# rokulkarni15/distributed-llm-training-inference

Measured on AMD Instinct MI355X. Metric: train tok/s Llama-2-7B ZeRO-3+LoRA at 1/2/4/8 GPUs; serve tok/s + p50 TTFT, higher is better.
Workload: dtype bf16

## Files before the change

### lumen/csrc/binding.cpp

```cpp
#include <torch/extension.h>
#include <c10/hip/HIPStream.h>
#include <hip/hip_runtime.h>

#include <algorithm>
#include <optional>
#include <stdexcept>
#include <string>
#include <vector>

extern "C" {
hipError_t lumen_rmsnorm_fwd(int, const void*, const void*, const void*, void*, void*, float*, int,
                             int, float, hipStream_t);
hipError_t lumen_rmsnorm_bwd(int, const void*, const void*, const void*, const float*, const void*,
                             void*, float*, int, int, hipStream_t);
hipError_t lumen_qkv_rope(int, int, void*, void*, void*, void*, const int*, const float*,
                          const float*, int, int, int, int, int, hipStream_t);
hipError_t lumen_rope_inplace(int, void*, const int*, const float*, const float*, int, int, int,
                              int, hipStream_t);
hipError_t lumen_swiglu(int, int, const void*, const void*, void*, int, int, int, int, hipStream_t);
hipError_t lumen_scale_dev(int, void*, long long, const float*, const float*, hipStream_t);
hipError_t lumen_cross_entropy(int, void*, const int64_t*, float*, float*, int, int, int, float,
                               int, const float*, hipStream_t);
hipError_t lumen_grad_norm_sq(int, const void*, long long, float*, hipStream_t);
hipError_t lumen_adamw(float*, int, const void*, float*, float*, int, void*, long long, float, float,
// ... 606 lines not shown
                    big.data_ptr(), ldb, small.data_ptr<float>(), lds, out.data_ptr(), cs0,
                    cs1, static_cast<float>(alpha), static_cast<int>(T), static_cast<int>(J),
                    static_cast<int>(split), static_cast<unsigned long long>(seed),
                    static_cast<unsigned int>(drop_thresh), static_cast<float>(drop_scale),
                    drop_ld, drop_col0, nseg, bo, so, oo, nc,
                    rope_cos ? rope_cos->data_ptr<float>() : nullptr,
                    rope_sin ? rope_sin->data_ptr<float>() : nullptr,
                    rope_pos ? rope_pos->data_ptr<int>() : nullptr, static_cast<int>(rope_mask),
                    cur_stream()),
        "lora2");
}

bool is_fp8(const at::Tensor& t) { return t.scalar_type() == at::kFloat8_e4m3fn; }

void need_cuda_f32(const at::Tensor& t, const char* what) {
  if (!t.is_cuda() || t.scalar_type() != at::kFloat)
    throw std::invalid_argument(std::string("lumen: ") + what + " must be an f32 GPU tensor");
}

void lora3_down(const at::Tensor& x, int64_t ldx, const at::Tensor& A, at::Tensor& Z, int64_t ldz,
                int64_t T, int64_t K, int64_t R, double alpha, int64_t seed, int64_t thresh,
                double drop_scale, int64_t drop_ld, int64_t drop_col0,
                const c10::optional<at::Tensor>& xe, int64_t xk, int64_t KP,
                const c10::optional<at::Tensor>& cnt, const c10::optional<at::Tensor>& slab) {
  if (!x.is_cuda()) throw std::invalid_argument("lumen: lora3_down needs GPU tensors");
  need_cuda_f32(A, "lora3_down A");
  need_cuda_f32(Z, "lora3_down Z");
  if (A.stride(1) != 1 || A.size(0) < R || A.size(1) < K || x.size(0) < T || Z.size(0) < T)
    throw std::invalid_argument("lumen: lora3_down shape mismatch");
  void* xp = nullptr;
  long long ldxe = 0;
  unsigned* cp = nullptr;
  if (xe && xe->defined()) {
    if (!cnt || !cnt->defined() || cnt->scalar_type() != at::kInt || !cnt->is_cuda() ||
        cnt->numel() < (T + 63) / 64 || xe->scalar_type() != x.scalar_type() || xe->dim() != 2 ||
        xe->stride(1) != 1 || xe->size(0) < T || xe->size(1) < xk + KP || Z.size(1) < R)
      throw std::invalid_argument("lumen: lora3_down fold tail: xe [T, >= xk + KP], cnt int32 [T / 64]");
    xp = xe->data_ptr();
    ldxe = xe->stride(0);
    cp = reinterpret_cast<unsigned*>(cnt->data_ptr<int>());
  }
  float* sp = nullptr;
  if (slab && slab->defined()) {
    const bool with_cnt = cnt && cnt->defined();
    if ((with_cnt && (cnt->scalar_type() != at::kInt || !cnt->is_cuda() ||
                      cnt->numel() < (T + 63) / 64)) ||
        slab->scalar_type() != at::kFloat || !slab->is_cuda() ||
        slab->numel() < ((T + 63) / 64) * ((K + 1023) / 1024) * 64 * R)
      throw std::invalid_argument("lumen: lora3_down slab / cnt too small");
    sp = slab->data_ptr<float>();
    cp = with_cnt ? reinterpret_cast<unsigned*>(cnt->data_ptr<int>()) : nullptr;
  }
  check(lumen_lora3_down(dcode(x), x.data_ptr(), ldx, A.data_ptr<float>(), A.stride(0),
                         Z.data_ptr<float>(), ldz, static_cast<int>(T), static_cast<int>(K),
                         static_cast<int>(R), static_cast<float>(alpha),
                         static_cast<unsigned long long>(seed), static_cast<unsigned int>(thresh),
                         static_cast<float>(drop_scale), drop_ld, drop_col0, xp, ldxe,
                         static_cast<int>(xk), static_cast<int>(KP), cp, sp, cur_stream()),
        "lora3_down");
}

void lora3_up(int64_t fwd, at::Tensor& out, int64_t ldo, const at::Tensor& s1, int64_t ld1,
              const at::Tensor& s2, int64_t ld2, int64_t T, int64_t J, double alpha, int64_t seed,
              int64_t thresh, double drop_scale, int64_t drop_ld, int64_t drop_col0,
              const std::vector<std::vector<int64_t>>& segs, const c10::optional<at::Tensor>& rope_cos,
              const c10::optional<at::Tensor>& rope_sin, const c10::optional<at::Tensor>& rope_pos,
              int64_t rope_mask) {
  if (!out.is_cuda()) throw std::invalid_argument("lumen: lora3_up needs GPU tensors");
  need_cuda_f32(s1, "lora3_up s1");
  need_cuda_f32(s2, "lora3_up s2");
  const int nseg = static_cast<int>(segs.size());
  if (nseg < 1 || nseg > 4) throw std::invalid_argument("lumen: lora3_up needs 1..4 segments");
  long long oo[4] = {0}, so1[4] = {0}, so2[4] = {0};
// ... 555 lines not shown
```

### lumen/csrc/kernels/lora_v3.hip

```cpp
#include "tile128.h"
#include "det.h"

namespace lumen {
namespace lv3 {

using namespace tile;

struct Drop {
  unsigned int seed, thresh;
  float scale;
  long long ld;
  long long col0;
};

__device__ __forceinline__ uint4 mask8(uint4 u, uint32_t keep) {
  const auto wm = [keep](int w) {
    return ((keep >> (2 * w)) & 1u ? 0x0000FFFFu : 0u) | ((keep >> (2 * w + 1)) & 1u ? 0xFFFF0000u : 0u);
  };
  return make_uint4(u.x & wm(0), u.y & wm(1), u.z & wm(2), u.w & wm(3));
}

template <typename T>
__device__ __forceinline__ uint4 ld_f32x8(const float* p, bool ok) {
  if (!ok) return make_uint4(0, 0, 0, 0);
  const float4 u = *reinterpret_cast<const float4*>(p);
  const float4 v = *reinterpret_cast<const float4*>(p + 4);
  return make_uint4(pk2<T>(u.x, u.y), pk2<T>(u.z, u.w), pk2<T>(v.x, v.y), pk2<T>(v.z, v.w));
}

struct DownArgs {
  const void* x; long long ldx;
  const float* A; long long lda;
// ... 325 lines not shown
    for (int i = 0; i < 4; ++i) ycur[i] = ynxt[i];
  }
}

struct DySeg {
  long long n_off[4], r_off[4], b_off[4];
  int n_len[4];
  int nseg;
};

struct DyArgs {
  const void* dy; long long ldy;
  const float* B; int r;
  const float* Z; long long ldz;
  float* dZ; long long lddz;
  float* dB;
  int T, TW;
  float alpha;
  DySeg seg;
  int probe;
  float* slab_z; float* slab_b;
  unsigned* cnt_z; unsigned* cnt_b;
};

constexpr int kDyCC = 2;

template <typename T>
__device__ __forceinline__ void dy_load(uint4 (&v)[4], const T* base, long long ld, int r0, int rmax,
                                        int c0, int cmax) {
#pragma unroll
  for (int i = 0; i < 4; ++i) {
    const int idx = threadIdx.x + i * 256;
    const int r = r0 + (idx >> 4), c = c0 + (idx & 15) * 8;
    const uint4 u = *reinterpret_cast<const uint4*>(base + (long long)min(r, rmax - 1) * ld +
                                                     min(c, cmax - 8));
    v[i] = (r < rmax && c < cmax) ? u : make_uint4(0, 0, 0, 0);
  }
}

__device__ __forceinline__ void dy_store(char* img, const uint4 (&v)[4]) {
#pragma unroll
  for (int i = 0; i < 4; ++i) {
    const int idx = threadIdx.x + i * 256;
    *reinterpret_cast<uint4*>(img + img_off_b(idx >> 4, idx & 15)) = v[i];
  }
}

template <typename T, int NJ>
__global__ void __launch_bounds__(256) dy3_kernel(DyArgs a) {
  __shared__ __attribute__((aligned(16))) char img[2][64 * 256];
  const int seg = blockIdx.z;
  const int NL = a.seg.n_len[seg];
  const int cb = blockIdx.x * 128 * kDyCC;
  const int tb = blockIdx.y * a.TW, te = min(a.T, tb + a.TW);
  if (cb >= NL || tb >= a.T) return;
  const int lane = threadIdx.x & 63, wid = threadIdx.x >> 6, L = lane & 15, g = lane >> 4;
  const T* dy = reinterpret_cast<const T*>(a.dy) + a.seg.n_off[seg];
  const float* B = a.B + a.seg.b_off[seg] * a.r;
  const float* Z = a.Z + a.seg.r_off[seg];
  float* dZ = a.dZ + a.seg.r_off[seg];
  float* dB = a.dB + a.seg.b_off[seg] * a.r;
  const int nch = min(kDyCC, (NL - cb + 127) / 128);

  uint4 bop[kDyCC][4][NJ];
#pragma unroll
  for (int cc = 0; cc < kDyCC; ++cc)
#pragma unroll
    for (int i = 0; i < 4; ++i)
#pragma unroll
      for (int jt = 0; jt < NJ; ++jt) {
        float f[8];
#pragma unroll
        for (int e = 0; e < 8; ++e) {
          const int c = cb + cc * 128 + 32 * i + 8 * g + e;
          const float u = B[(long long)min(c, NL - 1) * a.r + jt * 16 + L];
          f[e] = c < NL ? u : 0.f;
        }
        bop[cc][i][jt] = pack8<T>(f);
      }
  f32x4 dbacc[kDyCC][2][NJ];
#pragma unroll
  for (int cc = 0; cc < kDyCC; ++cc)
#pragma unroll
    for (int m = 0; m < 2; ++m)
#pragma unroll
      for (int jt = 0; jt < NJ; ++jt) dbacc[cc][m][jt] = f32x4{0.f, 0.f, 0.f, 0.f};

  const int nsub = (te - tb + 63) / 64;
  const int nstage = nsub * nch;
  uint4 v[4];
  dy_load<T>(v, dy, a.ldy, tb, te, cb, NL);
  int buf = 0;
  f32x4 dzacc[NJ];
  uint4 zop[2][NJ];
  for (int s = 0; s < nstage; ++s, buf ^= 1) {
    const int ts = s / nch, cc = s % nch;
    const int t0 = tb + ts * 64, cbase = cb + cc * 128;
    dy_store(img[buf], v);
    __syncthreads();
    float zf[2][NJ][8];
#pragma unroll
    for (int ks = 0; ks < 2; ++ks)
#pragma unroll
      for (int jt = 0; jt < NJ; ++jt)
#pragma unroll
        for (int e = 0; e < 8; ++e) {
          const int t = t0 + 32 * ks + 8 * g + e;
          zf[ks][jt][e] = Z[(long long)min(t, te - 1) * a.ldz + jt * 16 + L];
        }
    {
      const int s1 = min(s + 1, nstage - 1);
      const int ts1 = s1 / nch, cc1 = s1 % nch;
      dy_load<T>(v, dy, a.ldy, tb + ts1 * 64, te, cb + cc1 * 128, NL);
    }
    if (cc == 0) {
#pragma unroll
      for (int jt = 0; jt < NJ; ++jt) dzacc[jt] = f32x4{0.f, 0.f, 0.f, 0.f};
    }
    const char* im = img[buf];
#pragma unroll
    for (int i = 0; i < 4; ++i) {
      const uint4 av = row_read_b(im, wid * 16 + L, i * 4 + g);
#pragma unroll
      for (int c2 = 0; c2 < kDyCC; ++c2)
        if (c2 == cc) {
#pragma unroll
          for (int jt = 0; jt < NJ; ++jt) dzacc[jt] = Mfma<T>::run(av, bop[c2][i][jt], dzacc[jt]);
        }
    }
#pragma unroll
    for (int ks = 0; ks < 2; ++ks)
#pragma unroll
      for (int jt = 0; jt < NJ; ++jt) {
        float f[8];
#pragma unroll
        for (int e = 0; e < 8; ++e) f[e] = t0 + 32 * ks + 8 * g + e < te ? zf[ks][jt][e] : 0.f;
        zop[ks][jt] = pack8<T>(f);
      }
#pragma unroll
    for (int ks = 0; ks < 2; ++ks)
#pragma unroll
      for (int m = 0; m < 2; ++m) {
        const uint4 tv = tr_read_img_b(im, ks * 32, wid * 32 + m * 16, lane);
#pragma unroll
        for (int c2 = 0; c2 < kDyCC; ++c2)
          if (c2 == cc) {
#pragma unroll
            for (int jt = 0; jt < NJ; ++jt) dbacc[c2][m][jt] = Mfma<T>::run(tv, zop[ks][jt], dbacc[c2][m][jt]);
          }
      }
    if (cc == nch - 1) {
      if (a.slab_z != nullptr) {
        float* sz = a.slab_z + (((long long)seg * gridDim.y + blockIdx.y) * gridDim.x + blockIdx.x) *
                                   ((long long)a.TW * a.r);
#pragma unroll
        for (int jt = 0; jt < NJ; ++jt)
#pragma unroll
          for (int r = 0; r < 4; ++r) {
            const int t = t0 + wid * 16 + g * 4 + r;
            if (t < te) det::st_wt(sz + (long long)(t - tb) * a.r + jt * 16 + L, dzacc[jt][r]);
          }
      } else {
#pragma unroll
        for (int jt = 0; jt < NJ; ++jt)
#pragma unroll
          for (int r = 0; r < 4; ++r) {
            const int t = t0 + wid * 16 + g * 4 + r;
            if (t < te && (!(a.probe & 16) || dzacc[jt][r] == 1234.5f))
              atomicAdd(dZ + (long long)t * a.lddz + jt * 16 + L, a.alpha * dzacc[jt][r]);
          }
      }
    }
  }
  if (a.slab_z != nullptr) {
    float* sb = a.slab_b + (((long long)seg * gridDim.x + blockIdx.x) * gridDim.y + blockIdx.y) *
                               (256LL * a.r);
#pragma unroll
    for (int cc = 0; cc < kDyCC; ++cc) {
      if (cc >= nch) break;
#pragma unroll
      for (int m = 0; m < 2; ++m)
#pragma unroll
        for (int jt = 0; jt < NJ; ++jt)
#pragma unroll
          for (int r = 0; r < 4; ++r) {
            const int cl = cc * 128 + wid * 32 + m * 16 + g * 4 + r;
            if (cb + cl < NL) det::st_wt(sb + (long long)cl * a.r + jt * 16 + L, dbacc[cc][m][jt][r]);
          }
    }
    if (a.cnt_z == nullptr) return;
    __shared__ int lastf;
    const int ncb = (NL + 128 * kDyCC - 1) / (128 * kDyCC);
    const int J = NJ * 16;
    if (det::last_arriver(a.cnt_z + (long long)seg * gridDim.y + blockIdx.y, ncb, &lastf)) {
      const float* base = a.slab_z + ((long long)seg * gridDim.y + blockIdx.y) * gridDim.x *
                                         ((long long)a.TW * a.r);
      for (int i = threadIdx.x; i < (te - tb) * (J / 2); i += 256) {
        const int tl = i / (J / 2), j = (i % (J / 2)) * 2;
        const float2 v = det::sum_pairs(base + (long long)tl * a.r + j, (long long)a.TW * a.r, ncb);
        float* o = dZ + (long long)(tb + tl) * a.lddz + j;
        o[0] = a.alpha * v.x;
        o[1] = a.alpha * v.y;
      }
    }
    if (det::last_arriver(a.cnt_b + (long long)seg * gridDim.x + blockIdx.x, gridDim.y, &lastf)) {
      const float* base = a.slab_b + ((long long)seg * gridDim.x + blockIdx.x) * gridDim.y *
// ... 61 lines not shown
    const float2 v = sum_pairs_plain(base, (long long)a.TW * a.r, ncb);
    float* o = a.dZ + a.seg.r_off[seg] + t * a.lddz + j;
    o[0] = a.alpha * v.x;
    o[1] = a.alpha * v.y;
  } else {
    const long long c = i / hr;
    if (c >= NL) return;
    const int gx = (int)(c / (128 * kDyCC)), cl = (int)(c % (128 * kDyCC));
    const float* base = a.slab_b + (((long long)seg * gx_n + gx) * gy_n) * (256LL * a.r) +
                        (long long)cl * a.r + j;
    const float2 v = sum_pairs_plain(base, 256LL * a.r, gy_n);
    float* o = a.dB + (a.seg.b_off[seg] + c) * a.r + j;
    o[0] += a.alpha * v.x;
    o[1] += a.alpha * v.y;
  }
}

__global__ void __launch_bounds__(256) dxa3_reduce_kernel(const float* __restrict__ slab,
                                                          float* __restrict__ dA, long long ldda,
                                                          int R, int K, int gy_n, float scale) {
  const long long i = (long long)blockIdx.x * 256 + threadIdx.x;
  const int hk = K / 2;
  if (i >= (long long)R * hk) return;
  const int j = (int)(i / hk), k = (int)(i % hk) * 2;
  const int gx = k / 128, kl = k % 128;
  const float2 v = sum_pairs_plain(slab + ((long long)gx * gy_n) * (128LL * R) +
                                       (long long)j * 128 + kl,
                                   128LL * R, gy_n);
  float* o = dA + (long long)j * ldda + k;
  o[0] += scale * v.x;
  o[1] += scale * v.y;
}

__global__ void __launch_bounds__(256) down3_reduce_kernel(const float* __restrict__ slab,
                                                           float* __restrict__ Z, long long ldz,
                                                           int T, int J, int gy_n) {
  const long long i = (long long)blockIdx.x * 256 + threadIdx.x;
  const int hj = J / 2;
  if (i >= (long long)T * hj) return;
  const int t = (int)(i / hj), j = (int)(i % hj) * 2;
  const int tile = t / 64, row = t % 64;
  const float2 v = sum_pairs_plain(slab + ((long long)tile * gy_n) * (64LL * J) +
                                       (long long)row * J + j,
                                   64LL * J, gy_n);
  *reinterpret_cast<float2*>(Z + (long long)t * ldz + j) = v;
}

struct DxaArgs {
  const void* x; long long ldx;
  void* dx; long long lddx;
  const float* dZ;
  const float* A;
  long long lda;
  float* dA;
  long long ldda;
  int T, K, R, TW;
  float da_scale, dx_scale;
  Drop drop;
  int probe;
  float* slab; unsigned* cnt;
  float* delta;
};

constexpr int kDxST = 72;

template <typename T, bool DROP, int NJ, bool DELTA = false>
__global__ void __launch_bounds__(256) dxa3_kernel(DxaArgs a) {
  constexpr int J = NJ * 16, KJ = J > 32 ? 64 : 32, NKS = KJ / 32, SP = KJ + 8;
  __shared__ __attribute__((aligned(16))) char img[2][64 * 256];
  __shared__ __attribute__((aligned(16))) T st[2][J * kDxST];
  __shared__ __attribute__((aligned(16))) T s2[128 * SP];
  __shared__ uint8_t mk[DROP ? 2 : 1][DROP ? 64 * 16 : 1];
  const int c0 = blockIdx.x * 128;
  const int tb = blockIdx.y * a.TW, te = min(a.T, tb + a.TW);
  if (c0 >= a.K || tb >= a.T) return;
  const int lane = threadIdx.x & 63, wid = threadIdx.x >> 6, L = lane & 15, g = lane >> 4;
  const T* x = reinterpret_cast<const T*>(a.x);
  T* dx = reinterpret_cast<T*>(a.dx);
  constexpr int NS2 = 32 * KJ / 256;
  float4 f2[NS2];
#pragma unroll
  for (int q = 0; q < NS2; ++q) {
    const int idx = threadIdx.x + q * 256, j = idx / 32, c = (idx % 32) * 4;
    const int jj = min(j, a.R - 1), cc = min(c0 + c, a.K - 4);
    f2[q] = *reinterpret_cast<const float4*>(a.A + (long long)jj * a.lda + cc);
  }
#pragma unroll
  for (int q = 0; q < NS2; ++q) {
    const int idx = threadIdx.x + q * 256, j = idx / 32, c = (idx % 32) * 4;
    const bool ok = j < a.R && c0 + c < a.K;
    const float4 f = ok ? f2[q] : make_float4(0.f, 0.f, 0.f, 0.f);
    s2[(c + 0) * SP + j] = from_f32<T>(f.x);
    s2[(c + 1) * SP + j] = from_f32<T>(f.y);
    s2[(c + 2) * SP + j] = from_f32<T>(f.z);
    s2[(c + 3) * SP + j] = from_f32<T>(f.w);
  }
  f32x4 da[2][NJ];
#pragma unroll
  for (int m = 0; m < 2; ++m)
#pragma unroll
    for (int jt = 0; jt < NJ; ++jt) da[m][jt] = f32x4{0.f, 0.f, 0.f, 0.f};

  uint4 xv[4];
  float4 zv[(64 * J / 4 + 255) / 256];
  const auto load_stage = [&](int t0) {
#pragma unroll
    for (int i = 0; i < 4; ++i) {
      const int idx = threadIdx.x + i * 256;
      const int r = t0 + (idx >> 4), c = c0 + (idx & 15) * 8;
      const uint4 u = *reinterpret_cast<const uint4*>(x + (long long)min(r, te - 1) * a.ldx +
                                                       min(c, a.K - 8));
      xv[i] = (r < te && c < a.K) ? u : make_uint4(0, 0, 0, 0);
    }
#pragma unroll
    for (int i = 0; i < (64 * J / 4 + 255) / 256; ++i) {
      const int idx = threadIdx.x + i * 256;
      const int r = idx / (J / 4), j = (idx % (J / 4)) * 4;
      const float4 u = *reinterpret_cast<const float4*>(a.dZ + (long long)min(t0 + r, te - 1) * a.R + j);
      zv[i] = (r < 64 && t0 + r < te) ? u : make_float4(0.f, 0.f, 0.f, 0.f);
    }
  };
  const auto store_stage = [&](int t0, int b) {
#pragma unroll
    for (int i = 0; i < 4; ++i) {
      const int idx = threadIdx.x + i * 256;
      const int row = idx >> 4, ch = idx & 15;
      uint4 u = xv[i];
      if (DROP) {
        const uint32_t keep = dropout_keep8(
// ... 18 lines not shown
    }
  };
  float4 nbf[NKS][2];
  uint4 ndv[4];
  uint4 nov[DELTA ? 4 : 1];
  const auto load_rows = [&](int t0) {
    const int t = t0 + wid * 16 + L;
    const bool tok = t < te;
#pragma unroll
    for (int ks = 0; ks < NKS; ++ks) {
      const int j = min(ks * 32 + g * 8, a.R - 8);
      const float* zp = a.dZ + (long long)min(t, te - 1) * a.R + j;
      nbf[ks][0] = *reinterpret_cast<const float4*>(zp);
      nbf[ks][1] = *reinterpret_cast<const float4*>(zp + 4);
    }
    const long long tc = min(t, te - 1);
#pragma unroll
    for (int i = 0; i < 4; ++i) {
      const int c = c0 + 32 * i + 8 * g;
      const uint4 u = *reinterpret_cast<const uint4*>(dx + tc * a.lddx + min(c, a.K - 8));
      ndv[i] = (tok && c < a.K) ? u : make_uint4(0, 0, 0, 0);
    }
    if constexpr (DELTA) {
#pragma unroll
      for (int i = 0; i < 4; ++i) {
        const int c = c0 + 32 * i + 8 * g;
        const uint4 u = *reinterpret_cast<const uint4*>(x + tc * a.ldx + min(c, a.K - 8));
        nov[i] = (tok && c < a.K) ? u : make_uint4(0, 0, 0, 0);
      }
    }
  };
  load_stage(tb);
  load_rows(tb);
  int buf = 0;
  for (int t0 = tb; t0 < te; t0 += 64, buf ^= 1) {
    store_stage(t0, buf);
    __syncthreads();
    load_stage(t0 + 64);
    const int t = t0 + wid * 16 + L;
    const bool tok = t < te;
    uint4 bop[NKS], dv[4], ov[DELTA ? 4 : 1];
#pragma unroll
    for (int ks = 0; ks < NKS; ++ks) {
      const float4 u = nbf[ks][0], v = nbf[ks][1];
      bop[ks] = (tok && ks * 32 + g * 8 < a.R)
                    ? make_uint4(pk2<T>(u.x, u.y), pk2<T>(u.z, u.w), pk2<T>(v.x, v.y), pk2<T>(v.z, v.w))
                    : make_uint4(0, 0, 0, 0);
    }
#pragma unroll
    for (int i = 0; i < 4; ++i) dv[i] = ndv[i];
    if constexpr (DELTA) {
#pragma unroll
      for (int i = 0; i < 4; ++i) ov[i] = nov[i];
    }
    load_rows(t0 + 64);
    const char* im = img[buf];
    const T* sz = st[buf];
#pragma unroll
    for (int ks = 0; ks < 2; ++ks) {
      uint4 xt[2];
#pragma unroll
      for (int m = 0; m < 2; ++m) xt[m] = tr_read_img(im, ks * 32, wid * 32 + m * 16, lane);
#pragma unroll
      for (int jt = 0; jt < NJ; ++jt) {
        const uint4 zt = *reinterpret_cast<const uint4*>(sz + (jt * 16 + L) * kDxST + ks * 32 + g * 8);
#pragma unroll
// ... 120 lines not shown
  const int r = static_cast<int>(d[4]), K = static_cast<int>(d[3]);
  const int nch = r / 8;
  const long long i = static_cast<long long>(blockIdx.x) * 256 + threadIdx.x;
  const long long n_len = d[12 + seg];
  if (i >= n_len * nch) return;
  const long long n = i / nch;
  const int c = static_cast<int>(i % nch) * 8;
  const float scale = __builtin_bit_cast(float, static_cast<unsigned>(d[6]));
  const float* B = reinterpret_cast<const float*>(d[2]);
  T* w = reinterpret_cast<T*>(d[0]);
  float v[8];
  load8(B + (d[20 + seg] + n) * r + c, v);
#pragma unroll
  for (int e = 0; e < 8; ++e) v[e] *= scale;
  store8(w + (d[8 + seg] + n) * d[1] + K + d[16 + seg] + c, v);
}

}
}

using namespace lumen;

extern "C" hipError_t lumen_lora3_w_tail_batch(int dtype, const long long* desc, int n,
                                               long long max_chunks, hipStream_t st) {
  if (n <= 0 || max_chunks <= 0) return hipSuccess;
  if (n > 16383) return hipErrorInvalidValue;
  const dim3 grid(static_cast<unsigned>((max_chunks + 255) / 256), 4 * n), block(256);
  if (dtype == kBF16) hipLaunchKernelGGL(lv3::w_tail_batch_kernel<bf16>, grid, block, 0, st, desc);
  else if (dtype == kF16) hipLaunchKernelGGL(lv3::w_tail_batch_kernel<fp16>, grid, block, 0, st, desc);
  else return hipErrorInvalidValue;
  return hipGetLastError();
}

#include <cstdlib>
static int lv3_probe() {
  static int v = [] { const char* e = std::getenv("LUMEN_LV3_PROBE"); return e ? std::atoi(e) : 0; }();
  return v;
}

extern "C" hipError_t lumen_lora3_down(int dtype, const void* x, long long ldx, const float* A,
                                       long long lda, float* Z, long long ldz, int T, int K, int R,
                                       float alpha, unsigned long long seed, unsigned int thresh,
                                       float drop_scale, long long drop_ld, long long drop_col0,
                                       void* xe, long long ldxe, int xk, int KP, unsigned* cnt,
                                       float* slab, hipStream_t st) {
  if (T <= 0 || K <= 0 || R < 16 || R > 64 || (R & 15) || (K & 7) || (ldx & 7) || (lda & 3))
    return hipErrorInvalidValue;
  if (xe != nullptr && (cnt == nullptr || (KP & 7) || KP < R || (ldxe & 7) || (xk & 7)))
    return hipErrorInvalidValue;
  if (slab != nullptr && ((ldz & 1) || (cnt == nullptr && xe != nullptr)))
    return hipErrorInvalidValue;
  lv3::DownArgs a{x, ldx, A, lda, Z, ldz, T, K, alpha,
                  {static_cast<unsigned>(seed) ^ static_cast<unsigned>(seed >> 32), thresh, drop_scale,
                   drop_ld, drop_col0}, lv3_probe(), xe, ldxe, xk, KP, cnt, slab};
  const dim3 grid((T + 63) / 64, (K + 1023) / 1024), block(512);
  const bool drop = thresh != 0;
#define LV3_DOWN(TT, NJ)                                                                           \
  do {                                                                                           \
    if (drop) hipLaunchKernelGGL((lv3::down3_kernel<TT, true, NJ>), grid, block, 0, st, a);     \
    else hipLaunchKernelGGL((lv3::down3_kernel<TT, false, NJ>), grid, block, 0, st, a);         \
  } while (0)
#define LV3_DOWN_NJ(TT)                                                                            \
  switch (R / 16) {                                                                              \
    case 1: LV3_DOWN(TT, 1); break;                                                              \
    case 2: LV3_DOWN(TT, 2); break;                                                              \
    case 3: LV3_DOWN(TT, 3); break;                                                              \
    default: LV3_DOWN(TT, 4); break;                                                             \
  }
  if (dtype == kBF16) { LV3_DOWN_NJ(bf16) }
  else if (dtype == kF16) { LV3_DOWN_NJ(fp16) }
  else return hipErrorInvalidValue;
#undef LV3_DOWN_NJ
#undef LV3_DOWN
  if (slab != nullptr && cnt == nullptr) {
    const long long n = (long long)T * (R / 2);
    hipLaunchKernelGGL(lv3::down3_reduce_kernel, dim3((unsigned)((n + 255) / 256)), dim3(256), 0,
                       st, (const float*)slab, Z, ldz, T, R, (int)grid.y);
  }
  return hipGetLastError();
}

extern "C" hipError_t lumen_lora3_up(int dtype, int fwd, void* out, long long ldo, const float* s1,
                                     long long ld1, const float* s2, long long ld2, int T, int J,
                                     float alpha, unsigned long long seed, unsigned int thresh,
                                     float drop_scale, long long drop_ld, long long drop_col0,
                                     int nseg, const long long* out_off, const long long* s1_off,
                                     const long long* s2_off, const int* ncols,
                                     const float* rope_cos, const float* rope_sin,
                                     const int* rope_pos, int rope_mask, hipStream_t st) {
  if (T <= 0 || J < 1 || J > 64 || nseg < 1 || nseg > 4 || (ldo & 7) || (ld1 & 3) || (ld2 & 3))
    return hipErrorInvalidValue;
  lv3::UpArgs a;
  a.out = out; a.ldo = ldo; a.s1 = s1; a.ld1 = ld1; a.s2 = s2; a.ld2 = ld2; a.T = T; a.J = J;
  a.alpha = alpha;
  a.drop = {static_cast<unsigned>(seed) ^ static_cast<unsigned>(seed >> 32), thresh, drop_scale,
            drop_ld, drop_col0};
  a.seg.nseg = nseg;
  int maxc = 0;
  for (int i = 0; i < 4; ++i) {
    const bool v = i < nseg;
    a.seg.out_off[i] = v ? out_off[i] : 0; a.seg.s1_off[i] = v ? s1_off[i] : 0;
    a.seg.s2_off[i] = v ? s2_off[i] : 0; a.seg.ncols[i] = v ? ncols[i] : 0;
    if (v && ((ncols[i] & 7) || (out_off[i] & 7) || (s1_off[i] & 3))) return hipErrorInvalidValue;
    if (v && ncols[i] > maxc) maxc = ncols[i];
  }
  a.rope_cos = rope_cos; a.rope_sin = rope_sin; a.rope_pos = rope_pos;
  a.rope_mask = (fwd && rope_cos && rope_sin && rope_pos) ? rope_mask : 0;
  for (int i = 0; i < nseg; ++i)
    if (((a.rope_mask >> i) & 1) && ((out_off[i] & 127) || (ncols[i] & 127))) return hipErrorInvalidValue;
  if (maxc == 0) return hipSuccess;
  const dim3 grid((maxc + 127) / 128, (T + 64 * lv3::kUpRT - 1) / (64 * lv3::kUpRT), nseg), block(256);
  const bool drop = !fwd && thresh != 0;
#define LV3_UP(TT, KJ)                                                                             \
  do {                                                                                           \
    if (fwd) hipLaunchKernelGGL((lv3::up3_kernel<TT, true, false, KJ>), grid, block, 0, st, a);   \
    else if (drop) hipLaunchKernelGGL((lv3::up3_kernel<TT, false, true, KJ>), grid, block, 0, st, a); \
    else hipLaunchKernelGGL((lv3::up3_kernel<TT, false, false, KJ>), grid, block, 0, st, a);     \
  } while (0)
  if (dtype == kBF16) { if (J <= 32) LV3_UP(bf16, 32); else LV3_UP(bf16, 64); }
  else if (dtype == kF16) { if (J <= 32) LV3_UP(fp16, 32); else LV3_UP(fp16, 64); }
  else return hipErrorInvalidValue;
#undef LV3_UP
  return hipGetLastError();
}

extern "C" hipError_t lumen_lora3_dy(int dtype, const void* dy, long long ldy, const float* B, int r,
                                     const float* Z, long long ldz, float* dZ, long long lddz,
                                     float* dB, int T, int tw, float alpha, int nseg,
                                     const long long* n_off, const long long* r_off,
                                     const long long* b_off, const int* n_len, float* slab_z,
                                     float* slab_b, unsigned* cnt_z, unsigned* cnt_b,
                                     hipStream_t st) {
  if (T <= 0 || nseg < 1 || nseg > 4 || (r != 16 && r != 32 && r != 64) || tw < 64 || (tw & 63) ||
      (ldy & 7))
    return hipErrorInvalidValue;
  lv3::DyArgs a;
  a.probe = lv3_probe();
  a.dy = dy; a.ldy = ldy; a.B = B; a.r = r; a.Z = Z; a.ldz = ldz; a.dZ = dZ; a.lddz = lddz;
  a.dB = dB; a.T = T; a.TW = tw; a.alpha = alpha;
  a.slab_z = slab_z; a.slab_b = slab_b; a.cnt_z = cnt_z; a.cnt_b = cnt_b;
  if (slab_z != nullptr && (slab_b == nullptr || (cnt_z == nullptr) != (cnt_b == nullptr) ||
                            (lddz & 1)))
    return hipErrorInvalidValue;
  a.seg.nseg = nseg;
  int maxl = 0;
  for (int i = 0; i < 4; ++i) {
    const bool v = i < nseg;
    a.seg.n_off[i] = v ? n_off[i] : 0; a.seg.r_off[i] = v ? r_off[i] : 0;
    a.seg.b_off[i] = v ? b_off[i] : 0; a.seg.n_len[i] = v ? n_len[i] : 0;
    if (v && ((n_len[i] & 7) || (n_off[i] & 7))) return hipErrorInvalidValue;
    if (v && n_len[i] > maxl) maxl = n_len[i];
  }
  if (maxl == 0) return hipSuccess;
  const dim3 grid((maxl + 128 * lv3::kDyCC - 1) / (128 * lv3::kDyCC), (T + tw - 1) / tw, nseg), block(256);
#define LV3_DY(TT)                                                                                 \
  switch (r) {                                                                                   \
    case 16: hipLaunchKernelGGL((lv3::dy3_kernel<TT, 1>), grid, block, 0, st, a); break;          \
    case 32: hipLaunchKernelGGL((lv3::dy3_kernel<TT, 2>), grid, block, 0, st, a); break;          \
    default: hipLaunchKernelGGL((lv3::dy3_kernel<TT, 4>), grid, block, 0, st, a); break;          \
  }
  if (dtype == kBF16) { LV3_DY(bf16) }
  else if (dtype == kF16) { LV3_DY(fp16) }
  else return hipErrorInvalidValue;
#undef LV3_DY
  if (slab_z != nullptr && cnt_z == nullptr) {
    const long long n = (long long)(T > maxl ? T : maxl) * (r / 2);
    const dim3 rgrid((unsigned)((n + 255) / 256), nseg, 2);
    hipLaunchKernelGGL(lv3::dy3_reduce_kernel, rgrid, dim3(256), 0, st, a, (int)grid.x,
                       (int)grid.y);
  }
  return hipGetLastError();
}

extern "C" hipError_t lumen_lora3_z_tail(int dtype, const float* Z, int R, void* xe, long long ldx,
                                         int K, int KP, int T, hipStream_t st) {
  if (T <= 0) return hipSuccess;
  if ((KP & 7) || R > KP || (ldx & 7) || (K & 7)) return hipErrorInvalidValue;
  const long long n = static_cast<long long>(T) * (KP / 8);
  const dim3 grid(static_cast<unsigned>((n + 255) / 256)), block(256);
  if (dtype == kBF16) hipLaunchKernelGGL(lv3::z_tail_kernel<bf16>, grid, block, 0, st, Z, R, (bf16*)xe, ldx, K, KP, T);
  else if (dtype == kF16) hipLaunchKernelGGL(lv3::z_tail_kernel<fp16>, grid, block, 0, st, Z, R, (fp16*)xe, ldx, K, KP, T);
  else return hipErrorInvalidValue;
  return hipGetLastError();
// ... 83 lines not shown
```

### lumen/ops/lora.py

```python
from __future__ import annotations

import math
from typing import List, Optional, Sequence, Tuple

import torch
import torch.nn.functional as F

from ._native import DTYPE_CODE, native, use_native
from .gemm import mm_nt

Seg = Tuple[int, int, int, int]

_M32 = 0xFFFFFFFF


def _lowbias32(x):
    x = x ^ (x >> 16)
    x = (x * 0x7FEB352D) & _M32
    x = x ^ (x >> 15)
    x = (x * 0x846CA68B) & _M32
    x = x ^ (x >> 16)
    return x


# ... 119 lines not shown


USE_V3 = _os.environ.get("LUMEN_LORA_V3", "1") != "0"
DY_TW = int(_os.environ.get("LUMEN_LORA_DY_TW", "0"))
DXA_TW = int(_os.environ.get("LUMEN_LORA_DXA_TW", "0"))
DET_SPLIT = _os.environ.get("LUMEN_DET_SPLIT", "1") != "0"
DXA = _os.environ.get("LUMEN_LORA_DXA", "1") != "0"
DELTA_HANDOFF = _os.environ.get("LUMEN_FA_DELTA_HANDOFF", "1") != "0"
_DELTA_SLOT = [None]


DETERMINISTIC = _os.environ.get("LUMEN_LORA_DETERMINISTIC", "0") == "1"
_det: dict = {}


def _det_ws(dev, nfloat: int, ncnt: int):
    key = (str(dev), torch.cuda.current_stream(dev).cuda_stream)
    got = _det.get(key)
    if got is None or got[0].numel() < nfloat or got[1].numel() < ncnt:
        nf = max(nfloat, got[0].numel() if got is not None else 0, 1 << 20)
        nc = max(ncnt, got[1].numel() if got is not None else 0, 4096)
        got = (torch.empty(nf, dtype=torch.float32, device=dev),
               torch.zeros(nc, dtype=torch.int32, device=dev))
        _det[key] = got
    return got


def _v3_ok(r: int, R: int, segs, *mats) -> bool:
    return (USE_V3 and r in (16, 32, 64) and R % 16 == 0 and R <= 64
            and all(s[0] % 8 == 0 and s[1] % 8 == 0 for s in segs)
            and all(m.stride(1) == 1 and m.stride(0) % 8 == 0 for m in mats))


def _lora3_down(x2d, A, Z, p, seed):
    T, K = x2d.shape
    R = A.shape[0]
    cnt = slab = None
    if DETERMINISTIC and x2d.is_cuda:
        slab, cnt = _det_ws(x2d.device, math.ceil(T / 64) * math.ceil(K / 1024) * 64 * R,
                            math.ceil(T / 64))
    native().lora3_down(x2d, x2d.stride(0), A, Z, R, T, K, R, 1.0, int(seed) & 0x7FFFFFFFFFFFFFFF,
                        drop_threshold(p), 1.0 / (1.0 - p) if p > 0 else 1.0, K, 0,
                        None, 0, 0, None if (slab is not None and DET_SPLIT) else cnt, slab)


def _lora3_fwd(x2d, y, A, B, Z, segs, r, scale, p, seed, rope):
    _lora3_down(x2d, A, Z, p, seed)
    fuse = rope is not None and len(segs) <= 4 and _rope_covered(segs, rope[3])
    for i in range(0, len(segs), 4):
        ch = segs[i:i + 4]
        mask = sum(1 << j for j, sg in enumerate(ch) if sg[0] + sg[1] <= rope[3]) if fuse else 0
        _lora2(2, 1, B, Z, y, y.stride(0), 1, scale, T=x2d.shape[0], J=r, split=1,
               segs4=[(b_off * r, r_off, n_off, n_len) for (n_off, n_len, r_off, b_off) in ch],
               rope=(rope[1], rope[2], rope[0], mask) if fuse else None)
    return y, fuse


FOLD = _os.environ.get("LUMEN_LORA_FOLD", "1") != "0"
FOLD_KP = 64


def fold_operand(x2d: torch.Tensor, K: int) -> Optional[torch.Tensor]:
    if (x2d.dim() == 2 and x2d.shape[1] == K and x2d.stride(1) == 1
            and x2d.stride(0) == K + FOLD_KP and x2d.is_cuda):
        return x2d.as_strided((x2d.shape[0], K + FOLD_KP), (K + FOLD_KP, 1))
    return None


def _dy_tw(segs, T: int) -> int:
    if DY_TW:
        return DY_TW
    cols = sum(math.ceil(s[1] / 256) for s in segs)
    return 256 if cols * math.ceil(T / 256) >= 512 else 128


def lora_fwd_native(x2d, y, A, B, segs: Sequence[Seg], r, scale, p, seed, train: bool = False,
# ... 196 lines not shown

def _side_stream(dev) -> "torch.cuda.Stream":
    s = _side_streams.get(dev)
    if s is None:
        s = _side_streams[dev] = torch.cuda.Stream(device=dev)
    return s


def _direct_ok(prm: torch.Tensor) -> bool:
    g = prm.grad
    return (getattr(prm, "_lumen_direct_grad", False) and g is not None
            and g.dtype == torch.float32 and g.is_contiguous() and g.shape == prm.shape)



class _LoraLinear(torch.autograd.Function):
    @staticmethod
    def forward(ctx, x2d, weight_fn, bias, A, B, segs, r, scale, p, seed, w_param, wt_fn, train,
                rope, fold=None):
        ctx.train = train
        W = weight_fn() if fold is None else None

        def gemm():
            y_ = torch.matmul(x2d, W.t())
            if bias is not None:
                y_.add_(bias)
            return y_

        if fold is not None:
            T, K = x2d.shape
            R = A.shape[0]
            xe = fold_operand(x2d, K)
            Z = _zeros(T, R, device=x2d.device, train=ctx.train)
            _lora3_down(x2d, A, Z, p, seed)
            native().lora3_z_tail(Z, xe, K, FOLD_KP)
            y = torch.matmul(xe, fold.t())
            if bias is not None:
                y.add_(bias)
            rope_done = False
        else:
            y = gemm()
            Z, rope_done = lora_fwd_native(x2d, y, A, B, segs, r, scale, p, seed,
                                           train=ctx.train, rope=rope)
        if rope is not None and not rope_done:
            _rope_(y, rope, inverse=False)
        ctx.rope = rope
        ctx.delta_slot = getattr(x2d, "_lumen_delta_slot", None) if DELTA_HANDOFF else None
        ctx.weight_fn = weight_fn
        ctx.wt_fn = wt_fn
        ctx.meta = (segs, r, scale, p, seed)
        ctx.w_grad = w_param is not None and w_param.requires_grad
        ctx.b_grad = bias is not None and bias.requires_grad
        ctx.save_for_backward(x2d, A, B, Z)
        return y

    @staticmethod
    def backward(ctx, dy):
        x2d, A, B, Z = ctx.saved_tensors
        segs, r, scale, p, seed = ctx.meta
        dy = dy.contiguous()
        if ctx.rope is not None and not getattr(dy, "_lumen_rope_undone", False):
            if not getattr(dy, "_lumen_scratch", False):
                dy = dy.clone()
            _rope_(dy, ctx.rope, inverse=True)
        got = {}

        def dx_fn():
            got["dx"] = _input_grad(ctx, dy)
# ... 118 lines not shown
```

Measured before the change: 45040.

## Restage LoRA dy kernel through LDS and fuse fold tail into down pass

```diff
diff --git a/lumen/csrc/binding.cpp b/lumen/csrc/binding.cpp
--- a/lumen/csrc/binding.cpp
+++ b/lumen/csrc/binding.cpp
@@ -662,13 +662,15 @@
   long long ldxe = 0;
   unsigned* cp = nullptr;
   if (xe && xe->defined()) {
-    if (!cnt || !cnt->defined() || cnt->scalar_type() != at::kInt || !cnt->is_cuda() ||
-        cnt->numel() < (T + 63) / 64 || xe->scalar_type() != x.scalar_type() || xe->dim() != 2 ||
+    const bool split = slab && slab->defined() && !(cnt && cnt->defined());
+    if ((!split && (!cnt || !cnt->defined() || cnt->scalar_type() != at::kInt || !cnt->is_cuda() ||
+                    cnt->numel() < (T + 63) / 64)) ||
+        xe->scalar_type() != x.scalar_type() || xe->dim() != 2 ||
         xe->stride(1) != 1 || xe->size(0) < T || xe->size(1) < xk + KP || Z.size(1) < R)
       throw std::invalid_argument("lumen: lora3_down fold tail: xe [T, >= xk + KP], cnt int32 [T / 64]");
     xp = xe->data_ptr();
     ldxe = xe->stride(0);
-    cp = reinterpret_cast<unsigned*>(cnt->data_ptr<int>());
+    if (!split) cp = reinterpret_cast<unsigned*>(cnt->data_ptr<int>());
   }
   float* sp = nullptr;
   if (slab && slab->defined()) {
diff --git a/lumen/csrc/kernels/lora_v3.hip b/lumen/csrc/kernels/lora_v3.hip
--- a/lumen/csrc/kernels/lora_v3.hip
+++ b/lumen/csrc/kernels/lora_v3.hip
@@ -1,3 +1,5 @@
+#include <type_traits>
+
 #include "tile128.h"
 #include "det.h"
 
@@ -389,23 +391,30 @@
   for (int i = 0; i < 4; ++i) {
     const int idx = threadIdx.x + i * 256;
     const int r = r0 + (idx >> 4), c = c0 + (idx & 15) * 8;
-    const uint4 u = *reinterpret_cast<const uint4*>(base + (long long)min(r, rmax - 1) * ld +
-                                                     min(c, cmax - 8));
-    v[i] = (r < rmax && c < cmax) ? u : make_uint4(0, 0, 0, 0);
-  }
-}
-
-__device__ __forceinline__ void dy_store(char* img, const uint4 (&v)[4]) {
+    v[i] = *reinterpret_cast<const uint4*>(base + (long long)min(r, rmax - 1) * ld + min(c, cmax - 8));
+  }
+}
+
+__device__ __forceinline__ void dy_store(char* img, const uint4 (&v)[4], int r0, int rmax, int c0,
+                                         int cmax) {
 #pragma unroll
   for (int i = 0; i < 4; ++i) {
     const int idx = threadIdx.x + i * 256;
-    *reinterpret_cast<uint4*>(img + img_off_b(idx >> 4, idx & 15)) = v[i];
-  }
-}
+    const int r = r0 + (idx >> 4), c = c0 + (idx & 15) * 8;
+    *reinterpret_cast<uint4*>(img + img_off_b(idx >> 4, idx & 15)) =
+        (r < rmax && c < cmax) ? v[i] : make_uint4(0, 0, 0, 0);
+  }
+}
+
+constexpr int kDyBS = 264;
+constexpr int kDyZS = 72;
 
 template <typename T, int NJ>
-__global__ void __launch_bounds__(256) dy3_kernel(DyArgs a) {
-  __shared__ __attribute__((aligned(16))) char img[2][64 * 256];
+__global__ void __launch_bounds__(256, NJ == 1 ? 3 : 1) dy3_kernel(DyArgs a) {
+  constexpr int J = NJ * 16;
+  constexpr int kImg = 2 * 64 * 256, kBt = J * kDyBS * 2;
+  __shared__ __attribute__((aligned(16))) char smem[kImg > kBt ? kImg : kBt];
+  __shared__ __attribute__((aligned(16))) unsigned short zt[2][J * kDyZS];
   const int seg = blockIdx.z;
   const int NL = a.seg.n_len[seg];
   const int cb = blockIdx.x * 128 * kDyCC;
@@ -413,122 +422,159 @@
   if (cb >= NL || tb >= a.T) return;
   const int lane = threadIdx.x & 63, wid = threadIdx.x >> 6, L = lane & 15, g = lane >> 4;
   const T* dy = reinterpret_cast<const T*>(a.dy) + a.seg.n_off[seg];
-  const float* B = a.B + a.seg.b_off[seg] * a.r;
+  const float* B = a.B + a.seg.b_off[seg] * J;
   const float* Z = a.Z + a.seg.r_off[seg];
   float* dZ = a.dZ + a.seg.r_off[seg];
-  float* dB = a.dB + a.seg.b_off[seg] * a.r;
+  float* dB = a.dB + a.seg.b_off[seg] * J;
   const int nch = min(kDyCC, (NL - cb + 127) / 128);
-
-  uint4 bop[kDyCC][4][NJ];
-#pragma unroll
-  for (int cc = 0; cc < kDyCC; ++cc)
-#pragma unroll
-    for (int i = 0; i < 4; ++i)
-#pragma unroll
-      for (int jt = 0; jt < NJ; ++jt) {
-        float f[8];
-#pragma unroll
-        for (int e = 0; e < 8; ++e) {
-          const int c = cb + cc * 128 + 32 * i + 8 * g + e;
-          const float u = B[(long long)min(c, NL - 1) * a.r + jt * 16 + L];
-          f[e] = c < NL ? u : 0.f;
-        }
-        bop[cc][i][jt] = pack8<T>(f);
-      }
-  f32x4 dbacc[kDyCC][2][NJ];
-#pragma unroll
-  for (int cc = 0; cc < kDyCC; ++cc)
-#pragma unroll
-    for (int m = 0; m < 2; ++m)
-#pragma unroll
-      for (int jt = 0; jt < NJ; ++jt) dbacc[cc][m][jt] = f32x4{0.f, 0.f, 0.f, 0.f};
-
   const int nsub = (te - tb + 63) / 64;
   const int nstage = nsub * nch;
-  uint4 v[4];
-  dy_load<T>(v, dy, a.ldy, tb, te, cb, NL);
-  int buf = 0;
+
+  uint4 v[2][4];
+  const auto load_stage = [&](uint4 (&d)[4], int s) __attribute__((always_inline)) {
+    const int s1 = min(s, nstage - 1);
+    const int ts1 = nch == 2 ? s1 >> 1 : s1, cc1 = nch == 2 ? s1 & 1 : 0;
+    dy_load<T>(d, dy, a.ldy, tb + ts1 * 64, te, cb + cc1 * 128, NL);
+  };
+  float4 zq[NJ];
+  const auto z_load = [&](int t0) __attribute__((always_inline)) {
+#pragma unroll
+    for (int q = 0; q < NJ; ++q) {
+      const int idx = threadIdx.x + q * 256, row = idx / (J / 4), j = (idx % (J / 4)) * 4;
+      zq[q] = *reinterpret_cast<const float4*>(Z + (long long)min(t0 + row, te - 1) * a.ldz + j);
+    }
+  };
+  const auto z_store = [&](unsigned short* zs, int t0) __attribute__((always_inline)) {
+#pragma unroll
+    for (int q = 0; q < NJ; ++q) {
+      const int idx = threadIdx.x + q * 256, row = idx / (J / 4), j = (idx % (J / 4)) * 4;
+      const bool ok = t0 + row < te;
+      const unsigned u0 = ok ? pk2<T>(zq[q].x, zq[q].y) : 0u, u1 = ok ? pk2<T>(zq[q].z, zq[q].w) : 0u;
+      zs[(j + 0) * kDyZS + row] = static_cast<unsigned short>(u0);
+      zs[(j + 1) * kDyZS + row] = static_cast<unsigned short>(u0 >> 16);
+      zs[(j + 2) * kDyZS + row] = static_cast<unsigned short>(u1);
+      zs[(j + 3) * kDyZS + row] = static_cast<unsigned short>(u1 >> 16);
+    }
+  };
+
+  load_stage(v[0], 0);
+  load_stage(v[1], 1);
+  z_load(tb);
+  uint4 bop[kDyCC][4][NJ];
+  {
+    unsigned short* bt = reinterpret_cast<unsigned short*>(smem);
+    float4 bf[J / 4];
+#pragma unroll
+    for (int q = 0; q < J / 4; ++q) {
+      const int idx = threadIdx.x + q * 256, c = idx / (J / 4), j = (idx % (J / 4)) * 4;
+      bf[q] = *reinterpret_cast<const float4*>(B + (long long)min(cb + c, NL - 1) * J + j);
+    }
+#pragma unroll
+    for (int q = 0; q < J / 4; ++q) {
+      const int idx = threadIdx.x + q * 256, c = idx / (J / 4), j = (idx % (J / 4)) * 4;
+      const bool ok = cb + c < NL;
+      const unsigned u0 = ok ? pk2<T>(bf[q].x, bf[q].y) : 0u, u1 = ok ? pk2<T>(bf[q].z, bf[q].w) : 0u;
+      bt[(j + 0) * kDyBS + c] = static_cast<unsigned short>(u0);
+      bt[(j + 1) * kDyBS + c] = static_cast<unsigned short>(u0 >> 16);
+      bt[(j + 2) * kDyBS + c] = static_cast<unsigned short>(u1);
+      bt[(j + 3) * kDyBS + c] = static_cast<unsigned short>(u1 >> 16);
+    }
+    __syncthreads();
+#pragma unroll
+    for (int cc = 0; cc < kDyCC; ++cc)
+#pragma unroll
+      for (int i = 0; i < 4; ++i)
+#pragma unroll
+        for (int jt = 0; jt < NJ; ++jt)
+          bop[cc][i][jt] = *reinterpret_cast<const uint4*>(bt + (jt * 16 + L) * kDyBS + cc * 128 +
+                                                           32 * i + 8 * g);
+    __syncthreads();
+  }
+  f32x4 dbacc[kDyCC][2][NJ];
+#pragma unroll
+  for (int cc = 0; cc < kDyCC; ++cc)
+#pragma unroll
+    for (int m = 0; m < 2; ++m)
+#pragma unroll
+      for (int jt = 0; jt < NJ; ++jt) dbacc[cc][m][jt] = f32x4{0.f, 0.f, 0.f, 0.f};
   f32x4 dzacc[NJ];
-  uint4 zop[2][NJ];
-  for (int s = 0; s < nstage; ++s, buf ^= 1) {
-    const int ts = s / nch, cc = s % nch;
-    const int t0 = tb + ts * 64, cbase = cb + cc * 128;
-    dy_store(img[buf], v);
+
+  const auto flush_dz = [&](int t0) __attribute__((always_inline)) {
+    if (a.slab_z != nullptr) {
+      float* sz = a.slab_z + (((long long)seg * gridDim.y + blockIdx.y) * gridDim.x + blockIdx.x) *
+                                 ((long long)a.TW * J);
+#pragma unroll
+      for (int jt = 0; jt < NJ; ++jt)
+#pragma unroll
+        for (int r = 0; r < 4; ++r) {
+          const int t = t0 + wid * 16 + g * 4 + r;
+          if (t < te) det::st_wt(sz + (long long)(t - tb) * J + jt * 16 + L, dzacc[jt][r]);
+        }
+    } else {
+#pragma unroll
+      for (int jt = 0; jt < NJ; ++jt)
+#pragma unroll
+        for (int r = 0; r < 4; ++r) {
+          const int t = t0 + wid * 16 + g * 4 + r;
+          if (t < te && (!(a.probe & 16) || dzacc[jt][r] == 1234.5f))
+            atomicAdd(dZ + (long long)t * a.lddz + jt * 16 + L, a.alpha * dzacc[jt][r]);
+        }
+    }
+  };
+  const auto stage = [&](auto cc_, auto buf_, int s, int ts) __attribute__((always_inline)) {
+    constexpr int CC = decltype(cc_)::value, BUF = decltype(buf_)::value;
+    const int t0 = tb + ts * 64;
+    char* im = smem + BUF * (64 * 256);
+    const unsigned short* zs = zt[ts & 1];
+    dy_store(im, v[BUF], t0, te, cb + CC * 128, NL);
+    if (CC == 0) z_store(zt[ts & 1], t0);
     __syncthreads();
-    float zf[2][NJ][8];
-#pragma unroll
-    for (int ks = 0; ks < 2; ++ks)
-#pragma unroll
-      for (int jt = 0; jt < NJ; ++jt)
-#pragma unroll
-        for (int e = 0; e < 8; ++e) {
-          const int t = t0 + 32 * ks + 8 * g + e;
-          zf[ks][jt][e] = Z[(long long)min(t, te - 1) * a.ldz + jt * 16 + L];
-        }
-    {
-      const int s1 = min(s + 1, nstage - 1);
-      const int ts1 = s1 / nch, cc1 = s1 % nch;
-      dy_load<T>(v, dy, a.ldy, tb + ts1 * 64, te, cb + cc1 * 128, NL);
-    }
-    if (cc == 0) {
+    if (CC == 0) {
+      if (ts > 0) flush_dz(t0 - 64);
+      z_load(t0 + 64);
+    }
+    load_stage(v[BUF], s + 2);
+    if (CC == 0) {
 #pragma unroll
       for (int jt = 0; jt < NJ; ++jt) dzacc[jt] = f32x4{0.f, 0.f, 0.f, 0.f};
     }
-    const char* im = img[buf];
 #pragma unroll
     for (int i = 0; i < 4; ++i) {
       const uint4 av = row_read_b(im, wid * 16 + L, i * 4 + g);
 #pragma unroll
-      for (int c2 = 0; c2 < kDyCC; ++c2)
-        if (c2 == cc) {
-#pragma unroll
-          for (int jt = 0; jt < NJ; ++jt) dzacc[jt] = Mfma<T>::run(av, bop[c2][i][jt], dzacc[jt]);
-        }
-    }
+      for (int jt = 0; jt < NJ; ++jt) dzacc[jt] = Mfma<T>::run(av, bop[CC][i][jt], dzacc[jt]);
+    }
+    uint4 zop[2][NJ];
 #pragma unroll
     for (int ks = 0; ks < 2; ++ks)
 #pragma unroll
-      for (int jt = 0; jt < NJ; ++jt) {
-        float f[8];
-#pragma unroll
-        for (int e = 0; e < 8; ++e) f[e] = t0 + 32 * ks + 8 * g + e < te ? zf[ks][jt][e] : 0.f;
-        zop[ks][jt] = pack8<T>(f);
-      }
+      for (int jt = 0; jt < NJ; ++jt)
+        zop[ks][jt] = *reinterpret_cast<const uint4*>(zs + (jt * 16 + L) * kDyZS + 32 * ks + 8 * g);
 #pragma unroll
     for (int ks = 0; ks < 2; ++ks)
 #pragma unroll
       for (int m = 0; m < 2; ++m) {
         const uint4 tv = tr_read_img_b(im, ks * 32, wid * 32 + m * 16, lane);
 #pragma unroll
-        for (int c2 = 0; c2 < kDyCC; ++c2)
-          if (c2 == cc) {
-#pragma unroll
-            for (int jt = 0; jt < NJ; ++jt) dbacc[c2][m][jt] = Mfma<T>::run(tv, zop[ks][jt], dbacc[c2][m][jt]);
-          }
-      }
-    if (cc == nch - 1) {
-      if (a.slab_z != nullptr) {
-        float* sz = a.slab_z + (((long long)seg * gridDim.y + blockIdx.y) * gridDim.x + blockIdx.x) *
-                                   ((long long)a.TW * a.r);
-#pragma unroll
-        for (int jt = 0; jt < NJ; ++jt)
-#pragma unroll
-          for (int r = 0; r < 4; ++r) {
-            const int t = t0 + wid * 16 + g * 4 + r;
-            if (t < te) det::st_wt(sz + (long long)(t - tb) * a.r + jt * 16 + L, dzacc[jt][r]);
-          }
-      } else {
-#pragma unroll
-        for (int jt = 0; jt < NJ; ++jt)
-#pragma unroll
-          for (int r = 0; r < 4; ++r) {
-            const int t = t0 + wid * 16 + g * 4 + r;
-            if (t < te && (!(a.probe & 16) || dzacc[jt][r] == 1234.5f))
-              atomicAdd(dZ + (long long)t * a.lddz + jt * 16 + L, a.alpha * dzacc[jt][r]);
-          }
-      }
-    }
-  }
+        for (int jt = 0; jt < NJ; ++jt) dbacc[CC][m][jt] = Mfma<T>::run(tv, zop[ks][jt], dbacc[CC][m][jt]);
+      }
+  };
+  using I0 = std::integral_constant<int, 0>;
+  using I1 = std::integral_constant<int, 1>;
+  if (nch == 2) {
+    for (int ts = 0; ts < nsub; ++ts) {
+      stage(I0{}, I0{}, 2 * ts, ts);
+      stage(I1{}, I1{}, 2 * ts + 1, ts);
+    }
+  } else {
+    int ts = 0;
+    for (; ts + 1 < nsub; ts += 2) {
+      stage(I0{}, I0{}, ts, ts);
+      stage(I0{}, I1{}, ts + 1, ts + 1);
+    }
+    if (ts < nsub) stage(I0{}, I0{}, ts, ts);
+  }
+  flush_dz(tb + (nsub - 1) * 64);
   if (a.slab_z != nullptr) {
     float* sb = a.slab_b + (((long long)seg * gridDim.x + blockIdx.x) * gridDim.y + blockIdx.y) *
                                (256LL * a.r);
@@ -656,18 +702,25 @@
   o[1] += scale * v.y;
 }
 
+template <typename T>
 __global__ void __launch_bounds__(256) down3_reduce_kernel(const float* __restrict__ slab,
                                                            float* __restrict__ Z, long long ldz,
-                                                           int T, int J, int gy_n) {
+                                                           int T_, int J, int gy_n,
+                                                           T* __restrict__ xe, long long ldxe,
+                                                           int xk, int KP) {
   const long long i = (long long)blockIdx.x * 256 + threadIdx.x;
-  const int hj = J / 2;
-  if (i >= (long long)T * hj) return;
+  const int hj = (xe != nullptr && KP > J ? KP : J) / 2;
+  if (i >= (long long)T_ * hj) return;
   const int t = (int)(i / hj), j = (int)(i % hj) * 2;
-  const int tile = t / 64, row = t % 64;
-  const float2 v = sum_pairs_plain(slab + ((long long)tile * gy_n) * (64LL * J) +
-                                       (long long)row * J + j,
-                                   64LL * J, gy_n);
-  *reinterpret_cast<float2*>(Z + (long long)t * ldz + j) = v;
+  float2 v = make_float2(0.f, 0.f);
+  if (j < J) {
+    const int tile = t / 64, row = t % 64;
+    v = sum_pairs_plain(slab + ((long long)tile * gy_n) * (64LL * J) + (long long)row * J + j,
+                        64LL * J, gy_n);
+    *reinterpret_cast<float2*>(Z + (long long)t * ldz + j) = v;
+  }
+  if (xe != nullptr)
+    *reinterpret_cast<unsigned*>(xe + (long long)t * ldxe + xk + j) = pk2<T>(v.x, v.y);
 }
 
 struct DxaArgs {
@@ -701,24 +754,6 @@
   const int lane = threadIdx.x & 63, wid = threadIdx.x >> 6, L = lane & 15, g = lane >> 4;
   const T* x = reinterpret_cast<const T*>(a.x);
   T* dx = reinterpret_cast<T*>(a.dx);
-  constexpr int NS2 = 32 * KJ / 256;
-  float4 f2[NS2];
-#pragma unroll
-  for (int q = 0; q < NS2; ++q) {
-    const int idx = threadIdx.x + q * 256, j = idx / 32, c = (idx % 32) * 4;
-    const int jj = min(j, a.R - 1), cc = min(c0 + c, a.K - 4);
-    f2[q] = *reinterpret_cast<const float4*>(a.A + (long long)jj * a.lda + cc);
-  }
-#pragma unroll
-  for (int q = 0; q < NS2; ++q) {
-    const int idx = threadIdx.x + q * 256, j = idx / 32, c = (idx % 32) * 4;
-    const bool ok = j < a.R && c0 + c < a.K;
-    const float4 f = ok ? f2[q] : make_float4(0.f, 0.f, 0.f, 0.f);
-    s2[(c + 0) * SP + j] = from_f32<T>(f.x);
-    s2[(c + 1) * SP + j] = from_f32<T>(f.y);
-    s2[(c + 2) * SP + j] = from_f32<T>(f.z);
-    s2[(c + 3) * SP + j] = from_f32<T>(f.w);
-  }
   f32x4 da[2][NJ];
 #pragma unroll
   for (int m = 0; m < 2; ++m)
@@ -803,6 +838,24 @@
   };
   load_stage(tb);
   load_rows(tb);
+  constexpr int NS2 = 32 * KJ / 256;
+  float4 f2[NS2];
+#pragma unroll
+  for (int q = 0; q < NS2; ++q) {
+    const int idx = threadIdx.x + q * 256, j = idx / 32, c = (idx % 32) * 4;
+    const int jj = min(j, a.R - 1), cc = min(c0 + c, a.K - 4);
+    f2[q] = *reinterpret_cast<const float4*>(a.A + (long long)jj * a.lda + cc);
+  }
+#pragma unroll
+  for (int q = 0; q < NS2; ++q) {
+    const int idx = threadIdx.x + q * 256, j = idx / 32, c = (idx % 32) * 4;
+    const bool ok = j < a.R && c0 + c < a.K;
+    const float4 f = ok ? f2[q] : make_float4(0.f, 0.f, 0.f, 0.f);
+    s2[(c + 0) * SP + j] = from_f32<T>(f.x);
+    s2[(c + 1) * SP + j] = from_f32<T>(f.y);
+    s2[(c + 2) * SP + j] = from_f32<T>(f.z);
+    s2[(c + 3) * SP + j] = from_f32<T>(f.w);
+  }
   int buf = 0;
   for (int t0 = tb; t0 < te; t0 += 64, buf ^= 1) {
     store_stage(t0, buf);
@@ -989,6 +1042,7 @@
   return hipGetLastError();
 }
 
+#include <cstdint>
 #include <cstdlib>
 static int lv3_probe() {
   static int v = [] { const char* e = std::getenv("LUMEN_LV3_PROBE"); return e ? std::atoi(e) : 0; }();
@@ -1003,13 +1057,14 @@
                                        float* slab, hipStream_t st) {
   if (T <= 0 || K <= 0 || R < 16 || R > 64 || (R & 15) || (K & 7) || (ldx & 7) || (lda & 3))
     return hipErrorInvalidValue;
-  if (xe != nullptr && (cnt == nullptr || (KP & 7) || KP < R || (ldxe & 7) || (xk & 7)))
+  if (xe != nullptr && ((cnt == nullptr && slab == nullptr) || (KP & 7) || KP < R || (ldxe & 7) ||
+                        (xk & 7)))
     return hipErrorInvalidValue;
-  if (slab != nullptr && ((ldz & 1) || (cnt == nullptr && xe != nullptr)))
-    return hipErrorInvalidValue;
+  if (slab != nullptr && (ldz & 1)) return hipErrorInvalidValue;
+  const bool split = slab != nullptr && cnt == nullptr;
   lv3::DownArgs a{x, ldx, A, lda, Z, ldz, T, K, alpha,
                   {static_cast<unsigned>(seed) ^ static_cast<unsigned>(seed >> 32), thresh, drop_scale,
-                   drop_ld, drop_col0}, lv3_probe(), xe, ldxe, xk, KP, cnt, slab};
+                   drop_ld, drop_col0}, lv3_probe(), split ? nullptr : xe, ldxe, xk, KP, cnt, slab};
   const dim3 grid((T + 63) / 64, (K + 1023) / 1024), block(512);
   const bool drop = thresh != 0;
 #define LV3_DOWN(TT, NJ)                                                                           \
@@ -1029,10 +1084,15 @@
   else return hipErrorInvalidValue;
 #undef LV3_DOWN_NJ
 #undef LV3_DOWN
-  if (slab != nullptr && cnt == nullptr) {
-    const long long n = (long long)T * (R / 2);
-    hipLaunchKernelGGL(lv3::down3_reduce_kernel, dim3((unsigned)((n + 255) / 256)), dim3(256), 0,
-                       st, (const float*)slab, Z, ldz, T, R, (int)grid.y);
+  if (split) {
+    const long long n = (long long)T * ((xe != nullptr && KP > R ? KP : R) / 2);
+    const dim3 rgrid((unsigned)((n + 255) / 256));
+    if (dtype == kBF16)
+      hipLaunchKernelGGL(lv3::down3_reduce_kernel<bf16>, rgrid, dim3(256), 0, st, (const float*)slab,
+                         Z, ldz, T, R, (int)grid.y, (bf16*)xe, ldxe, xk, KP);
+    else
+      hipLaunchKernelGGL(lv3::down3_reduce_kernel<fp16>, rgrid, dim3(256), 0, st, (const float*)slab,
+                         Z, ldz, T, R, (int)grid.y, (fp16*)xe, ldxe, xk, KP);
   }
   return hipGetLastError();
 }
@@ -1091,6 +1151,8 @@
   if (T <= 0 || nseg < 1 || nseg > 4 || (r != 16 && r != 32 && r != 64) || tw < 64 || (tw & 63) ||
       (ldy & 7))
     return hipErrorInvalidValue;
+  if ((ldz & 3) || (reinterpret_cast<uintptr_t>(Z) & 15) || (reinterpret_cast<uintptr_t>(B) & 15))
+    return hipErrorInvalidValue;
   lv3::DyArgs a;
   a.probe = lv3_probe();
   a.dy = dy; a.ldy = ldy; a.B = B; a.r = r; a.Z = Z; a.ldz = ldz; a.dZ = dZ; a.lddz = lddz;
@@ -1105,7 +1167,7 @@
     const bool v = i < nseg;
     a.seg.n_off[i] = v ? n_off[i] : 0; a.seg.r_off[i] = v ? r_off[i] : 0;
     a.seg.b_off[i] = v ? b_off[i] : 0; a.seg.n_len[i] = v ? n_len[i] : 0;
-    if (v && ((n_len[i] & 7) || (n_off[i] & 7))) return hipErrorInvalidValue;
+    if (v && ((n_len[i] & 7) || (n_off[i] & 7) || (r_off[i] & 3))) return hipErrorInvalidValue;
     if (v && n_len[i] > maxl) maxl = n_len[i];
   }
   if (maxl == 0) return hipSuccess;
diff --git a/lumen/ops/lora.py b/lumen/ops/lora.py
--- a/lumen/ops/lora.py
+++ b/lumen/ops/lora.py
@@ -175,16 +175,31 @@
             and all(m.stride(1) == 1 and m.stride(0) % 8 == 0 for m in mats))
 
 
-def _lora3_down(x2d, A, Z, p, seed):
+_tail_cnt: dict = {}
+
+
+def _tail_counters(dev, n: int) -> torch.Tensor:
+    key = (str(dev), torch.cuda.current_stream(dev).cuda_stream)
+    got = _tail_cnt.get(key)
+    if got is None or got.numel() < n:
+        got = _tail_cnt[key] = torch.zeros(max(n, 4096), dtype=torch.int32, device=dev)
+    return got
+
+
+def _lora3_down(x2d, A, Z, p, seed, xe=None, xk=0, KP=0):
     T, K = x2d.shape
     R = A.shape[0]
     cnt = slab = None
     if DETERMINISTIC and x2d.is_cuda:
         slab, cnt = _det_ws(x2d.device, math.ceil(T / 64) * math.ceil(K / 1024) * 64 * R,
                             math.ceil(T / 64))
+        if DET_SPLIT:
+            cnt = None
+    elif xe is not None:
+        cnt = _tail_counters(x2d.device, math.ceil(T / 64))
     native().lora3_down(x2d, x2d.stride(0), A, Z, R, T, K, R, 1.0, int(seed) & 0x7FFFFFFFFFFFFFFF,
                         drop_threshold(p), 1.0 / (1.0 - p) if p > 0 else 1.0, K, 0,
-                        None, 0, 0, None if (slab is not None and DET_SPLIT) else cnt, slab)
+                        xe, xk, KP, cnt, slab)
 
 
 def _lora3_fwd(x2d, y, A, B, Z, segs, r, scale, p, seed, rope):
@@ -447,8 +462,7 @@
             R = A.shape[0]
             xe = fold_operand(x2d, K)
             Z = _zeros(T, R, device=x2d.device, train=ctx.train)
-            _lora3_down(x2d, A, Z, p, seed)
-            native().lora3_z_tail(Z, xe, K, FOLD_KP)
+            _lora3_down(x2d, A, Z, p, seed, xe, K, FOLD_KP)
             y = torch.matmul(xe, fold.t())
             if bias is not None:
                 y.add_(bias)
```

New measurement: 45110, median of 6. No clear change (+0.2%).
